# EndlessReform/smoltts

Hardware: AMD Instinct MI355X
Metric: Mimi frames/sec (=12.5 x RTF), greedy DualAR decode + Mimi decode to PCM (higher is better)
Workload: dtype bf16 weights, fp32 activations/accumulate, fp32 KV cache (LM); fp32 (Mimi)

## Files before the change

### smoltts_amd/csrc/seanet.hip

```cpp
#include "gemm_dev.h"
#include "mimi_common.h"

namespace smoltts {

namespace {

struct ResDev {
  const float* x;
  long x_bstride;
  int T;
  const char* w2;
  const float* b2;
  const char* w3;
  const float* b3;
  float* out;
  long o_bstride;
};

__device__ __forceinline__ float elu_fast(float x) { return x > 0.f ? x : __expf(x) - 1.0f; }

template <int C, int RC, int NW>
struct ResCfg {
  static constexpr int H = C / 2, RT = RC, RL = RC + 2, RLP = (RL + 15) / 16 * 16;
  static constexpr int CC = C / 32, HC = H / 32, K2C = 3 * CC;
  static constexpr int NT2 = H / 16, NT3 = C / 16, MT = RC / 16;
  static constexpr int WR = MT < NW ? MT : NW, WC = NW / WR;
  static constexpr int HP_U4 = 3 * CC * 4 * RLP, VP_U4 = 3 * HC * 4 * RC;
  static constexpr int GK3 = 1;
  static constexpr int WB_BYTES = NT3 * 3072 > 12288 ? NT3 * 3072 : 12288;
  static constexpr int GK2 = (WB_BYTES / (NT2 * 3072)) >= K2C ? K2C : ((WB_BYTES / (NT2 * 3072)) >= 2 ? 2 : 1);
  static constexpr size_t LDS = (size_t)(HP_U4 + VP_U4) * 16 + WB_BYTES;
  static_assert(MT % WR == 0 && NW % WR == 0 && NT2 % WC == 0 && NT3 % WC == 0, "wave arrangement");
  static_assert(K2C % GK2 == 0 && NT2 * GK2 * 3072 <= WB_BYTES && NT3 * GK3 * 3072 <= WB_BYTES, "weight groups");
};

template <int C, int RC, int NW, int NP>
__global__ __launch_bounds__(NW * 64) void resblock_kernel(ResDev p) {
  using K = ResCfg<C, RC, NW>;
  constexpr int NTHR = NW * 64;
  constexpr int H = K::H, RT = K::RT, RL = K::RL, RLP = K::RLP, CC = K::CC, HC = K::HC, K2C = K::K2C;
  constexpr int NT2 = K::NT2, NT3 = K::NT3, MT = K::MT, WR = K::WR, WC = K::WC;
  extern __shared__ __attribute__((aligned(16))) char smem[];
  uint4* hp = reinterpret_cast<uint4*>(smem);
  uint4* vp = hp + K::HP_U4;
  uint4* wb = vp + K::VP_U4;
  const int tid = threadIdx.x, wave = tid >> 6, lane = tid & 63;
  const int r = lane & 15, q = lane >> 4;
  const int b = blockIdx.y;
  const int u0 = blockIdx.x * RT;
  const int cu0 = u0;
  const float* xb = p.x + (long)b * p.x_bstride;
  const int wr = wave % WR, wc = wave / WR;

  constexpr int WPT = (K::WB_BYTES / 16 + NTHR - 1) / NTHR;
  uint4 wreg[WPT];
#define ST_FETCH_W(WSRC, NT, KC, K0, GK)                                                                          \
  _Pragma("unroll") for (int t_ = 0; t_ < WPT; ++t_) {                                                            \
    const int j_ = tid + t_ * NTHR;                                                                               \
    const int blk_ = j_ / 192, rem_ = j_ - blk_ * 192, nt_ = blk_ / (GK), kcl_ = blk_ - nt_ * (GK);              \
    wreg[t_] = j_ < (NT) * (GK) * 192                                                                             \
                   ? *reinterpret_cast<const uint4*>((WSRC) + (size_t)(nt_ * (KC) + (K0) + kcl_) * 3072 + rem_ * 16) \
                   : make_uint4(0, 0, 0, 0);                                                                      \
  }
#define ST_STORE_W(NT, GK)                                                                                        \
  _Pragma("unroll") for (int t_ = 0; t_ < WPT; ++t_) {                                                            \
    const int j_ = tid + t_ * NTHR;                                                                               \
    if (j_ < (NT) * (GK) * 192) wb[j_] = wreg[t_];                                                                \
  }

  ST_FETCH_W(p.w2, NT2, K2C, 0, K::GK2)
  for (int idx = tid; idx < (RL + 7) / 8 * 8 * (C / 8); idx += NTHR) {
    const int lr = idx / (C / 8 * 8) * 8 + (idx & 7), g8 = (idx >> 3) % (C / 8);
    if (lr >= RL) continue;
    const int row = cu0 - 2 + lr;
    float4 a = make_float4(0.f, 0.f, 0.f, 0.f), c = a;
    if (row < p.T) {
      const float* src = xb + (long)row * C + g8 * 8;
      a = *reinterpret_cast<const float4*>(src);
      c = *reinterpret_cast<const float4*>(src + 4);
    }
    a = make_float4(elu_fast(a.x), elu_fast(a.y), elu_fast(a.z), elu_fast(a.w));
    c = make_float4(elu_fast(c.x), elu_fast(c.y), elu_fast(c.z), elu_fast(c.w));
    uint4 h, m, l;
    split3x8(a, c, h, m, l);
    const int slot = ((g8 >> 2) * 4 + (g8 & 3)) * RLP + lr;
    hp[slot] = h;
    hp[slot + CC * 4 * RLP] = m;
    hp[slot + 2 * CC * 4 * RLP] = l;
  }
  ST_STORE_W(NT2, K::GK2)
  __syncthreads();

  {
    constexpr int RW = MT / WR, CW = NT2 / WC, G2 = K2C / K::GK2;
    f32x4 acc[RW][CW];
#pragma unroll
    for (int i = 0; i < RW; ++i)
#pragma unroll
      for (int j = 0; j < CW; ++j) acc[i][j] = (f32x4){0.f, 0.f, 0.f, 0.f};
    for (int g = 0; g < G2; ++g) {
      if (g + 1 < G2) {
        ST_FETCH_W(p.w2, NT2, K2C, (g + 1) * K::GK2, K::GK2)
      } else {
        ST_FETCH_W(p.w3, NT3, HC, 0, K::GK3)
      }
#pragma unroll
      for (int kcl = 0; kcl < K::GK2; ++kcl) {
        const int kc = g * K::GK2 + kcl, tap = kc / CC, xc = kc - tap * CC;
#pragma unroll
        for (int i = 0; i < RW; ++i) {
          const int mt = wr + i * WR;
          uint4 xf[3];
#pragma unroll
          for (int pc = 0; pc < 3; ++pc) xf[pc] = hp[((pc * CC + xc) * 4 + q) * RLP + mt * 16 + r + tap];
#pragma unroll
          for (int j = 0; j < CW; ++j) {
            uint4 wf[3];
#pragma unroll
            for (int pc = 0; pc < 3; ++pc) wf[pc] = wb[(((wc * CW + j) * K::GK2 + kcl) * 3 + pc) * 64 + lane];
            acc[i][j] = mfma_b3<NP>(wf, xf, acc[i][j]);
          }
        }
      }
      __syncthreads();
      if (g + 1 < G2) {
        ST_STORE_W(NT2, K::GK2)
        __syncthreads();
      } else {
        ST_STORE_W(NT3, K::GK3)
      }
    }
    uint2* vp2 = reinterpret_cast<uint2*>(vp);
#pragma unroll
    for (int i = 0; i < RW; ++i)
#pragma unroll
      for (int j = 0; j < CW; ++j) {
        const int row = (wr + i * WR) * 16 + r, ct = wc * CW + j, n = ct * 16 + 4 * q;
        const float4 bb = *reinterpret_cast<const float4*>(p.b2 + n);
        const float v0 = elu_fast(acc[i][j][0] + bb.x), v1 = elu_fast(acc[i][j][1] + bb.y), v2 = elu_fast(acc[i][j][2] + bb.z),
                    v3 = elu_fast(acc[i][j][3] + bb.w);
        uint32_t h0, m0, l0, h1, m1, l1;
        split3_pair(v0, v1, h0, m0, l0);
        split3_pair(v2, v3, h1, m1, l1);
        const int hc = ct >> 1, qv = (ct & 1) * 2 + (q >> 1);
        const int s2 = ((hc * 4 + qv) * RC + row) * 2 + (q & 1);
        vp2[s2] = make_uint2(h0, h1);
        vp2[s2 + HC * 4 * RC * 2] = make_uint2(m0, m1);
        vp2[s2 + 2 * HC * 4 * RC * 2] = make_uint2(l0, l1);
      }
    __syncthreads();
  }

  {
    constexpr int RW = MT / WR, CW = NT3 / WC, G3 = HC / K::GK3;
    f32x4 acc[RW][CW];
    float4 xres[RW][CW];
#pragma unroll
    for (int i = 0; i < RW; ++i) {
      const int grow = cu0 + (wr + i * WR) * 16 + r;
#pragma unroll
      for (int j = 0; j < CW; ++j) {
        acc[i][j] = (f32x4){0.f, 0.f, 0.f, 0.f};
        xres[i][j] = grow < p.T ? *reinterpret_cast<const float4*>(xb + (long)grow * C + (wc * CW + j) * 16 + 4 * q) : make_float4(0.f, 0.f, 0.f, 0.f);
      }
    }
    for (int g = 0; g < G3; ++g) {
      if (g + 1 < G3) {
        ST_FETCH_W(p.w3, NT3, HC, (g + 1) * K::GK3, K::GK3)
      }
#pragma unroll
      for (int kcl = 0; kcl < K::GK3; ++kcl) {
        const int kc = g * K::GK3 + kcl;
#pragma unroll
        for (int i = 0; i < RW; ++i) {
          const int mt = wr + i * WR;
          uint4 xf[3];
#pragma unroll
          for (int pc = 0; pc < 3; ++pc) xf[pc] = vp[((pc * HC + kc) * 4 + q) * RC + mt * 16 + r];
#pragma unroll
          for (int j = 0; j < CW; ++j) {
            uint4 wf[3];
#pragma unroll
            for (int pc = 0; pc < 3; ++pc) wf[pc] = wb[(((wc * CW + j) * K::GK3 + kcl) * 3 + pc) * 64 + lane];
            acc[i][j] = mfma_b3<NP>(wf, xf, acc[i][j]);
          }
        }
      }
      if (g + 1 < G3) {
        __syncthreads();
        ST_STORE_W(NT3, K::GK3)
        __syncthreads();
      }
    }
#pragma unroll
    for (int i = 0; i < RW; ++i) {
      const int row = (wr + i * WR) * 16 + r, grow = cu0 + row;
#pragma unroll
      for (int j = 0; j < CW; ++j) {
        const int n = (wc * CW + j) * 16 + 4 * q;
        float4 e = make_float4(0.f, 0.f, 0.f, 0.f);
        if (grow < p.T) {
          const float4 bb = *reinterpret_cast<const float4*>(p.b3 + n), xr = xres[i][j];
          e = make_float4(elu_fast(acc[i][j][0] + bb.x + xr.x), elu_fast(acc[i][j][1] + bb.y + xr.y), elu_fast(acc[i][j][2] + bb.z + xr.z),
                          elu_fast(acc[i][j][3] + bb.w + xr.w));
        }
        if (grow < p.T) *reinterpret_cast<float4*>(p.out + (long)b * p.o_bstride + (long)grow * C + n) = e;
      }
    }
  }

#undef ST_FETCH_W
#undef ST_STORE_W

}

template <int C, int RC, int NW, int NP>
int launch_res(const ResDev& d, int batch, hipStream_t st) {
  using K = ResCfg<C, RC, NW>;
  static PerDevice attr;
  const int dev = PerDevice::current();
  if (!attr.done(dev)) {
    ST_CHECK_HIP(hipFuncSetAttribute((const void*)resblock_kernel<C, RC, NW, NP>, hipFuncAttributeMaxDynamicSharedMemorySize, (int)K::LDS));
    attr.mark_done(dev);
  }
  const dim3 grid((d.T + K::RT - 1) / K::RT, batch);
  ST_REQUIRE(grid.y <= 65535, SMOLTTS_E_INVALID, "resblock: batch too large");
  hipLaunchKernelGGL((resblock_kernel<C, RC, NW, NP>), grid, dim3(NW * 64), K::LDS, st, d);
  ST_CHECK_HIP(hipGetLastError());
  return SMOLTTS_OK;
}

}

int launch_seanet_resblock(const MimiResblockArgs& a, hipStream_t st) {
  ST_REQUIRE(a.x && a.w2 && a.b2 && a.w3 && a.b3 && a.out && a.T > 0 && a.batch > 0, SMOLTTS_E_INVALID, "resblock: null or empty argument");
  ResDev d{a.x, (long)a.x_bstride, a.T, (const char*)a.w2, a.b2, (const char*)a.w3, a.b3, a.out, (long)a.o_bstride};
  if (a.channels == 128) return a.b3_products == 3 ? launch_res<128, 32, 8, 3>(d, a.batch, st) : launch_res<128, 32, 8, 6>(d, a.batch, st);
  set_error("resblock: no instance for %d channels", a.channels);
  return SMOLTTS_E_INVALID;
}

}
```

Measured before the change: 28750.

## Add persistent SEANet resblock kernel with register-resident weights and prefetch

New measurement: 28710, median of 6. No clear change (-0.1%).

```diff
diff --git a/smoltts_amd/csrc/seanet.hip b/smoltts_amd/csrc/seanet.hip
--- a/smoltts_amd/csrc/seanet.hip
+++ b/smoltts_amd/csrc/seanet.hip
@@ -230,14 +230,189 @@
   return SMOLTTS_OK;
 }
 
+constexpr int RP = 64, RP_W = 4, RP_THR = RP_W * 64;
+typedef unsigned u32x4r __attribute__((ext_vector_type(4)));
+__device__ __forceinline__ float4 ld_rows(__amdgpu_buffer_rsrc_t rs, unsigned off) {
+  const u32x4r v = __builtin_amdgcn_raw_buffer_load_b128(rs, off, 0, 0);
+  return make_float4(__uint_as_float(v[0]), __uint_as_float(v[1]), __uint_as_float(v[2]), __uint_as_float(v[3]));
+}
+
+template <int NP>
+__global__ __launch_bounds__(RP_THR) __attribute__((amdgpu_waves_per_eu(1, 1))) void resblock_persistent_kernel(ResDev p, int tiles_per_slot, int n_tiles) {
+  constexpr int C = 128, H = C / 2, CC = C / 32, HC = H / 32, K2C = 3 * CC, MT = RP / 16;
+  constexpr int RL = RP + 2, RLP = (RL + 15) / 16 * 16;
+  constexpr int HP_U4 = 3 * CC * 4 * RLP;
+  constexpr int NPW = NP == 6 ? 3 : 2;
+  constexpr int IN_ITEMS = (RL + 7) / 8 * 8 * (C / 8), IN_IT = (IN_ITEMS + RP_THR - 1) / RP_THR;
+  extern __shared__ __attribute__((aligned(16))) char smem[];
+  uint4* hp = reinterpret_cast<uint4*>(smem);
+  uint4* vp = hp + HP_U4;
+  const int tid = threadIdx.x, lane = tid & 63;
+  const int wave = __builtin_amdgcn_readfirstlane(tid >> 6);
+  const int r = lane & 15, q = lane >> 4;
+
+  uint4 w2r[K2C][3], w3r[2][HC][3];
+#pragma unroll
+  for (int kc = 0; kc < K2C; ++kc)
+#pragma unroll
+    for (int pc = 0; pc < NPW; ++pc) w2r[kc][pc] = *reinterpret_cast<const uint4*>(p.w2 + ((size_t)(wave * K2C + kc) * 3 + pc) * 1024 + lane * 16);
+#pragma unroll
+  for (int j = 0; j < 2; ++j)
+#pragma unroll
+    for (int kc = 0; kc < HC; ++kc)
+#pragma unroll
+      for (int pc = 0; pc < NPW; ++pc)
+        w3r[j][kc][pc] = *reinterpret_cast<const uint4*>(p.w3 + ((size_t)((2 * wave + j) * HC + kc) * 3 + pc) * 1024 + lane * 16);
+  const float4 b2r = *reinterpret_cast<const float4*>(p.b2 + wave * 16 + 4 * q);
+  float4 b3r[2];
+#pragma unroll
+  for (int j = 0; j < 2; ++j) b3r[j] = *reinterpret_cast<const float4*>(p.b3 + (2 * wave + j) * 16 + 4 * q);
+
+  auto x_rows = [&](int tile) {
+    const int fb = tile / tiles_per_slot;
+    return __builtin_amdgcn_make_buffer_rsrc((void*)(p.x + (long)fb * p.x_bstride - 2 * C), 0, tile < n_tiles ? (p.T + 2) * C * 4 : 0, 0x00020000);
+  };
+  float4 pre[IN_IT][2];
+  auto fetch = [&](int tile) {
+    const __amdgpu_buffer_rsrc_t rs = x_rows(tile);
+    const int fu0 = (tile - tile / tiles_per_slot * tiles_per_slot) * RP;
+#pragma unroll
+    for (int it = 0; it < IN_IT; ++it) {
+      const int idx = tid + RP_THR * it, lr = (idx >> 7) * 8 + (idx & 7), g8 = (idx >> 3) & 15;
+      const unsigned off = (unsigned)(((fu0 + lr) * C + g8 * 8) * 4);
+      pre[it][0] = ld_rows(rs, off);
+      pre[it][1] = ld_rows(rs, off + 16);
+    }
+  };
+  fetch(blockIdx.x);
+  __builtin_amdgcn_s_waitcnt(0xF70);
+
+  for (int tile = blockIdx.x; tile < n_tiles; tile += gridDim.x) {
+    const int b = tile / tiles_per_slot, u0 = (tile - b * tiles_per_slot) * RP;
+    const __amdgpu_buffer_rsrc_t xs = x_rows(tile);
+    const __amdgpu_buffer_rsrc_t os = __builtin_amdgcn_make_buffer_rsrc((void*)(p.out + (long)b * p.o_bstride), 0, p.T * C * 4, 0x00020000);
+
+#pragma unroll
+    for (int it = 0; it < IN_IT; ++it) {
+      const int idx = tid + RP_THR * it, lr = (idx >> 7) * 8 + (idx & 7), g8 = (idx >> 3) & 15;
+      if (idx >= IN_ITEMS || lr >= RL) continue;
+      const float4 a = make_float4(elu_fast(pre[it][0].x), elu_fast(pre[it][0].y), elu_fast(pre[it][0].z), elu_fast(pre[it][0].w));
+      const float4 c = make_float4(elu_fast(pre[it][1].x), elu_fast(pre[it][1].y), elu_fast(pre[it][1].z), elu_fast(pre[it][1].w));
+      uint4 h, m, l;
+      split3x8(a, c, h, m, l);
+      const int slot = g8 * RLP + lr;
+      hp[slot] = h;
+      hp[slot + CC * 4 * RLP] = m;
+      if (NP == 6) hp[slot + 2 * CC * 4 * RLP] = l;
+    }
+    lds_barrier();
+    fetch(tile + gridDim.x);
+
+    float4 xres[MT][2];
+#pragma unroll
+    for (int mt = 0; mt < MT; ++mt) {
+      const int grow = u0 + mt * 16 + r;
+#pragma unroll
+      for (int j = 0; j < 2; ++j) xres[mt][j] = ld_rows(xs, (unsigned)(((grow + 2) * C + (2 * wave + j) * 16 + 4 * q) * 4));
+    }
+
+    {
+      f32x4 acc[MT];
+#pragma unroll
+      for (int mt = 0; mt < MT; ++mt) acc[mt] = (f32x4){0.f, 0.f, 0.f, 0.f};
+#pragma unroll
+      for (int kc = 0; kc < K2C; ++kc) {
+        const int tap = kc / CC, xc = kc - tap * CC;
+#pragma unroll
+        for (int mt = 0; mt < MT; ++mt) {
+          uint4 xf[3];
+#pragma unroll
+          for (int pc = 0; pc < NPW; ++pc) xf[pc] = hp[((pc * CC + xc) * 4 + q) * RLP + mt * 16 + r + tap];
+          acc[mt] = mfma_b3<NP>(w2r[kc], xf, acc[mt]);
+        }
+      }
+      uint2* vp2 = reinterpret_cast<uint2*>(vp);
+      const int ct = wave, hc = ct >> 1, qv = (ct & 1) * 2 + (q >> 1);
+#pragma unroll
+      for (int mt = 0; mt < MT; ++mt) {
+        const int row = mt * 16 + r;
+        const float v0 = elu_fast(acc[mt][0] + b2r.x), v1 = elu_fast(acc[mt][1] + b2r.y), v2 = elu_fast(acc[mt][2] + b2r.z),
+                    v3 = elu_fast(acc[mt][3] + b2r.w);
+        uint32_t h0, m0, l0, h1, m1, l1;
+        split3_pair(v0, v1, h0, m0, l0);
+        split3_pair(v2, v3, h1, m1, l1);
+        const int s2 = ((hc * 4 + qv) * RP + row) * 2 + (q & 1);
+        vp2[s2] = make_uint2(h0, h1);
+        vp2[s2 + HC * 4 * RP * 2] = make_uint2(m0, m1);
+        if (NP == 6) vp2[s2 + 2 * HC * 4 * RP * 2] = make_uint2(l0, l1);
+      }
+    }
+    lds_barrier();
+
+    {
+      f32x4 acc[MT][2];
+#pragma unroll
+      for (int mt = 0; mt < MT; ++mt)
+#pragma unroll
+        for (int j = 0; j < 2; ++j) acc[mt][j] = (f32x4){0.f, 0.f, 0.f, 0.f};
+#pragma unroll
+      for (int kc = 0; kc < HC; ++kc)
+#pragma unroll
+        for (int mt = 0; mt < MT; ++mt) {
+          uint4 xf[3];
+#pragma unroll
+          for (int pc = 0; pc < NPW; ++pc) xf[pc] = vp[((pc * HC + kc) * 4 + q) * RP + mt * 16 + r];
+#pragma unroll
+          for (int j = 0; j < 2; ++j) acc[mt][j] = mfma_b3<NP>(w3r[j][kc], xf, acc[mt][j]);
+        }
+#pragma unroll
+      for (int mt = 0; mt < MT; ++mt) {
+        const int grow = u0 + mt * 16 + r;
+#pragma unroll
+        for (int j = 0; j < 2; ++j) {
+          const int n = (2 * wave + j) * 16 + 4 * q;
+          const float4 bb = b3r[j], xr = xres[mt][j];
+          u32x4r e;
+          e[0] = __float_as_uint(elu_fast(acc[mt][j][0] + bb.x + xr.x));
+          e[1] = __float_as_uint(elu_fast(acc[mt][j][1] + bb.y + xr.y));
+          e[2] = __float_as_uint(elu_fast(acc[mt][j][2] + bb.z + xr.z));
+          e[3] = __float_as_uint(elu_fast(acc[mt][j][3] + bb.w + xr.w));
+          __builtin_amdgcn_raw_buffer_store_b128(e, os, (unsigned)((grow * C + n) * 4), 0, 0);
+        }
+      }
+    }
+  }
+}
+
+constexpr size_t RP_LDS = (size_t)(3 * 4 * 4 * ((RP + 2 + 15) / 16 * 16) + 3 * 2 * 4 * RP) * 16;
+
+template <int NP>
+int launch_res_persistent(const ResDev& d, int batch, hipStream_t st) {
+  static PerDevice attr;
+  const int dev = PerDevice::current();
+  if (!attr.done(dev)) {
+    ST_CHECK_HIP(hipFuncSetAttribute((const void*)resblock_persistent_kernel<NP>, hipFuncAttributeMaxDynamicSharedMemorySize, (int)RP_LDS));
+    attr.mark_done(dev);
+  }
+  const int tiles_per_slot = (d.T + RP - 1) / RP;
+  ST_REQUIRE((long)tiles_per_slot * batch < (1L << 30) && (long)(d.T + RP + 2) * 128 * 4 < (1L << 31), SMOLTTS_E_INVALID,
+             "resblock: too many rows for one launch");
+  const int n_tiles = tiles_per_slot * batch, n_cu = device_cu_count();
+  const dim3 grid(n_tiles < n_cu ? n_tiles : n_cu);
+  hipLaunchKernelGGL((resblock_persistent_kernel<NP>), grid, dim3(RP_THR), RP_LDS, st, d, tiles_per_slot, n_tiles);
+  ST_CHECK_HIP(hipGetLastError());
+  return SMOLTTS_OK;
+}
+
 }
 
 int launch_seanet_resblock(const MimiResblockArgs& a, hipStream_t st) {
   ST_REQUIRE(a.x && a.w2 && a.b2 && a.w3 && a.b3 && a.out && a.T > 0 && a.batch > 0, SMOLTTS_E_INVALID, "resblock: null or empty argument");
   ResDev d{a.x, (long)a.x_bstride, a.T, (const char*)a.w2, a.b2, (const char*)a.w3, a.b3, a.out, (long)a.o_bstride};
-  if (a.channels == 128) return a.b3_products == 3 ? launch_res<128, 32, 8, 3>(d, a.batch, st) : launch_res<128, 32, 8, 6>(d, a.batch, st);
-  set_error("resblock: no instance for %d channels", a.channels);
-  return SMOLTTS_E_INVALID;
-}
-
-}
+  ST_REQUIRE(a.channels == 128, SMOLTTS_E_INVALID, "resblock: no instance for %d channels", a.channels);
+  static const bool tiled = ST_KNOB_INT("SMOLTTS_RESBLOCK_TILED", 0) != 0;
+  if (tiled) return a.b3_products == 3 ? launch_res<128, 32, 8, 3>(d, a.batch, st) : launch_res<128, 32, 8, 6>(d, a.batch, st);
+  return a.b3_products == 3 ? launch_res_persistent<3>(d, a.batch, st) : launch_res_persistent<6>(d, a.batch, st);
+}
+
+}
```
